# iamwangyabin/hardnetNas

Measured on AMD Instinct MI355X. Metric: Mpatches/s (32×32→128-D) at 1/2/4/8 MI355X; HPatches FPR95 parity, higher is better.
Workload: dtype bf16x3; 1 GPU; Stock HardNet forward, 262144 synthetic 32x32 patches per GPU; model=hardnet, global_batch=262144, per_gpu_batch=262144, parallelism=dp1

## Files before the change

### hardnetnas_amd/csrc/hn_api.hip

```cpp
#include "hardnet_mi355x.h"
#include "hn_internal.h"

#include <algorithm>
#include <cmath>
#include <cstdlib>
#include <cstring>
#include <map>
#include <mutex>
#include <string>
#include <utility>
#include <vector>

static thread_local std::string g_err;

static int env_int(const char* name, int dflt) {
  const char* e = std::getenv(name);
  return e ? std::atoi(e) : dflt;
}

void hn_read_knobs(HnKnobs* k) {
  *k = HnKnobs{};
  k->c12_cfg = env_int("HN_C12_CFG", 15);
  k->head = std::getenv("HN_HEAD_V1") ? 1 : env_int("HN_HEAD", 4);
  k->head_pf = env_int("HN_HEAD_PF", 1) != 0;
  k->fdl_valu = std::getenv("HN_FDL_VALU") != nullptr;
  k->naive_pw = std::getenv("HN_NAIVE_PW") != nullptr;
  k->naive_dw = std::getenv("HN_NAIVE_DW") != nullptr;
  k->no_skipfuse = std::getenv("HN_NO_SKIPFUSE") != nullptr;
  k->no_irfskip = std::getenv("HN_NO_IRFSKIP") != nullptr;
  k->pairdist_valu = std::getenv("HN_PAIRDIST_VALU") != nullptr;
  k->pairdist_reg = env_int("HN_PAIRDIST_REG", 0) != 0;
  k->pairdist_spread = env_int("HN_PAIRDIST_SPREAD", 1) != 0;
  k->front_fold = env_int("HN_FRONT_FOLD", 0) != 0;
  k->u8_apart = env_int("HN_U8_APART", 0) != 0;
  k->front_xch3 = env_int("HN_FRONT_XCH3", 0) != 0;
  k->no_mpfront = env_int("HN_NO_MPFRONT", 0) != 0;
  k->pipeline = env_int("HN_PIPELINE", 0) != 0;

  k->train_splitk = std::max(32, env_int("HN_TRAIN_SPLITK", 1024)) / 32 * 32;
  k->train_f32 = env_int("HN_TRAIN_F32", 17) & 255;
#ifdef HN_EXPERIMENTS
  k->c12_abl = env_int("HN_C12_ABL", 0) & 4095;
  k->c12w_pd = env_int("HN_C12W_PD", 11);
  k->dbg = env_int("HN_DEBUG", 0);
  k->head_abl = env_int("HN_HEAD_ABL", 0);
  k->w4_abl = env_int("HN_W4_ABL", 0);
  k->pairdist_abl = env_int("HN_PAIRDIST_ABL", 0);
  k->irf3 = env_int("HN_IRF3", 0) != 0;
#endif
}

static thread_local const HnKnobs* tl_knobs = nullptr;

const HnKnobs& hn_knobs() {
  if (tl_knobs) return *tl_knobs;
  static std::once_flag once;
  static HnKnobs process;
  std::call_once(once, [] { hn_read_knobs(&process); });
  return process;
}

namespace {
struct KnobScope {
  const HnKnobs* prev;
  explicit KnobScope(const HnKnobs* k) : prev(tl_knobs) { tl_knobs = k; }
  ~KnobScope() { tl_knobs = prev; }
};
}

hipError_t hn_resident_blocks(const void* fn, int nthreads, int lds, int* resident) {
  static std::mutex mu;
  static std::map<std::pair<const void*, int>, int> cache;
  int dev = 0;
  hipError_t e = hipGetDevice(&dev);
// ... 159 lines not shown
  bool c12 = true;
  int subchunk = 65536;
  int c12group = 65536;
  int c4sub = 0;
  uint16_t* front_spack = nullptr;
  int front = 0;
  bool no_front = false;
  bool no_irf = false;
  bool no_irf2 = false;
  const HnConvRow* conv[6] = {};
  size_t ws_floats_per_patch = 0;
  int n_bufs = 0;
  hipStream_t st2 = nullptr;
  hipEvent_t ev_fork = nullptr, ev_ready[2] = {nullptr, nullptr}, ev_free[2] = {nullptr, nullptr};
  std::mutex pipe_mu;

  template <class T>
  int upload(const std::vector<T>& v, T** out) {
    void* d = nullptr;
    if (hipMalloc(&d, v.size() * sizeof(T)) != hipSuccess)
      return fail(HN_ERR_NOMEM, "hipMalloc of parameters failed");
    allocs.push_back(d);
    HIPCHK(hipMemcpy(d, v.data(), v.size() * sizeof(T), hipMemcpyHostToDevice));
    *out = static_cast<T*>(d);
    return HN_OK;
  }
  ~hn_model() {
    for (void* p : allocs) (void)hipFree(p);
    for (hipEvent_t e : {ev_fork, ev_ready[0], ev_ready[1], ev_free[0], ev_free[1]})
      if (e) (void)hipEventDestroy(e);
    if (st2) (void)hipStreamDestroy(st2);
  }
};

static int check_desc(const hn_arch_desc* d) {
  if (!d) return fail(HN_ERR_ARG, "desc is NULL");
  if (d->kind == HN_KIND_HARDNET) return HN_OK;
  const bool fdl = d->kind == HN_KIND_FDL_NASNET || d->kind == HN_KIND_FDL_NASNET01;
  if (d->kind != HN_KIND_NAS && !fdl) return fail(HN_ERR_ARG, "unknown desc->kind");
  if (d->n_layers < 1 || d->n_layers > HN_MAX_LAYERS)
    return fail(HN_ERR_ARG, "n_layers out of range");
  int hw = fdl ? 8 : 32, c = fdl ? 64 : 32;
  for (int i = 0; i < d->n_layers; ++i) {
    if (d->op[i] < 0 || d->op[i] >= 17) return fail(HN_ERR_ARG, "op index out of range");
    if (d->c_in[i] != c) return fail(HN_ERR_ARG, "c_in does not chain");
    if (d->stride[i] != 1 && d->stride[i] != 2) return fail(HN_ERR_ARG, "stride must be 1/2");
    if (d->c_out[i] % 4 || d->c_in[i] % 4 || d->c_out[i] > 256)
      return fail(HN_ERR_ARG, "channel counts must be multiples of 4 and <= 256");
// ... 588 lines not shown
  (void)hipGetDevice(&m->device);
  Cursor cur{host_params, n_params};
  tl_f16_out_of_range = 0;
  rc = desc->kind == HN_KIND_HARDNET ? build_hardnet(m, cur)
       : desc->kind == HN_KIND_NAS    ? build_nas(m, cur)
                                      : build_fdl(m, cur);
  if (!rc && cur.i != n_params) rc = fail(HN_ERR_ARG, "host_params not fully consumed");
  if (!rc && tl_f16_out_of_range)
    rc = fail(HN_ERR_ARG, std::to_string(tl_f16_out_of_range) +
                              " BN-folded weights are outside the fp16 range of the fp16x3 kernels (|w| >= 65520 "
                              "or not finite)");
  if (rc) {
    delete m;
    return rc;
  }
  *out = m;
  return HN_OK;
}

static bool hardnet_subchunked(const hn_model* m) {
  return m->desc.kind == HN_KIND_HARDNET && m->c12 && !m->unfused_stem;
}
static int64_t hardnet_sub(const hn_model* m, int64_t p) { return std::max<int64_t>(1, std::min<int64_t>(p, m->subchunk)); }
static int64_t hardnet_group(const hn_model* m, int64_t p) {
  return std::max(hardnet_sub(m, p), std::min<int64_t>(p, m->c12group));
}
static size_t hardnet_a3_floats(const hn_model* m, int64_t p) {
  return std::max((size_t)16384 * hardnet_sub(m, p), (size_t)8192 * std::min<int64_t>(p, kHeadSplitMaxP));
}

// ... 262 lines not shown
extern "C" int hn_forward(hn_model* m, const float* d_in, int64_t batch, float* d_out,
                          void* d_workspace, size_t workspace_bytes, void* hip_stream) {
  if (!m) return fail(HN_ERR_ARG, "model is NULL");
  if (batch < 0) return fail(HN_ERR_ARG, "negative batch");
  if (batch == 0) return HN_OK;
  if (!d_in || !d_out || !d_workspace) return fail(HN_ERR_ARG, "NULL device pointer");
  if ((reinterpret_cast<uintptr_t>(d_in) | reinterpret_cast<uintptr_t>(d_out) |
       reinterpret_cast<uintptr_t>(d_workspace)) & 15)
    return fail(HN_ERR_ARG, "device pointers must be 16-byte aligned");
  size_t need = 0;
  hn_workspace_bytes(m, batch, &need);
  if (workspace_bytes < need)
    return fail(HN_ERR_WORKSPACE, "workspace too small: need " + std::to_string(need) + " bytes");
  hipStream_t st = static_cast<hipStream_t>(hip_stream);
  KnobScope knobs(&m->knobs);
  if (hardnet_pipelined(m, batch)) return forward_hardnet_pipe(m, d_in, batch, d_out, static_cast<float*>(d_workspace), st);
  for (int64_t off = 0; off < batch; off += m->chunk) {
    const int P = (int)std::min<int64_t>(m->chunk, batch - off);
    const float* in = d_in + off * 1024;
    float* out = d_out + off * 128;
    float* ws = static_cast<float*>(d_workspace);
    const int pmax = (int)std::min<int64_t>(m->chunk, batch);
    const int rc = m->desc.kind == HN_KIND_HARDNET ? forward_hardnet(m, in, P, pmax, out, ws, st)
                                                   : forward_nas(m, in, P, pmax, out, ws, st);
    if (rc) return rc;
  }
  return HN_OK;
}

static bool u8_fused(const hn_model* m, int resize) {
// ... 25 lines not shown
  if (in_hw != want)
    return fail(HN_ERR_ARG, "in_hw must be " + std::to_string(want) + " for this resize mode, got " +
                                std::to_string(in_hw));
  if (normalize && !(stdv != 0.0f)) return fail(HN_ERR_ARG, "std must be nonzero");
  if (batch == 0) return HN_OK;
  if (!d_in || !d_out || !d_workspace) return fail(HN_ERR_ARG, "NULL device pointer");
  if ((reinterpret_cast<uintptr_t>(d_in) | reinterpret_cast<uintptr_t>(d_out) |
       reinterpret_cast<uintptr_t>(d_workspace)) & 15)
    return fail(HN_ERR_ARG, "device pointers must be 16-byte aligned");
  size_t need = 0;
  hn_workspace_bytes_u8(m, batch, &need);
  if (workspace_bytes < need)
    return fail(HN_ERR_WORKSPACE, "workspace too small: need " + std::to_string(need) + " bytes");
  hipStream_t st = static_cast<hipStream_t>(hip_stream);
  KnobScope knobs(&m->knobs);
  const bool fused = u8_fused(m, resize);
  const size_t inb = (size_t)in_hw * in_hw;
  float* ws = static_cast<float*>(d_workspace);
  size_t base = 0;
  hn_workspace_bytes(m, batch, &base);
  float* pre = reinterpret_cast<float*>(static_cast<char*>(d_workspace) + base);
  const int pmax = (int)std::min<int64_t>(m->chunk, batch);
  for (int64_t off = 0; off < batch; off += m->chunk) {
    const int P = (int)std::min<int64_t>(m->chunk, batch - off);
    const uint8_t* in = d_in + off * inb;
    float* out = d_out + off * 128;
    int rc;
    if (fused) {
      const HnU8In u8{in, resize, normalize, mean, stdv};
      rc = m->desc.kind == HN_KIND_HARDNET ? forward_hardnet(m, nullptr, P, pmax, out, ws, st, &u8)
// ... 41 lines not shown
                             const int64_t* d_kpts, const float* d_scale, const float* d_ori, const float* d_ratio,
                             int64_t n, float* d_out, void* d_workspace, size_t workspace_bytes, void* hip_stream) {
  if (const char* e = clip_arg_error(n_images, height, width, n)) return fail(HN_ERR_ARG, e);
  if (!m) return fail(HN_ERR_ARG, "model is NULL");
  if (n == 0) return HN_OK;
  if (!d_images || !d_kpts || !d_scale || !d_ratio || !d_out || !d_workspace)
    return fail(HN_ERR_ARG, "NULL device pointer (only d_ori may be NULL)");
  if ((reinterpret_cast<uintptr_t>(d_out) | reinterpret_cast<uintptr_t>(d_workspace)) & 15)
    return fail(HN_ERR_ARG, "d_out / d_workspace must be 16-byte aligned");
  size_t need = 0, base = 0;
  hn_workspace_bytes_kp(m, n, &need);
  if (workspace_bytes < need)
    return fail(HN_ERR_WORKSPACE, "workspace too small: need " + std::to_string(need) + " bytes");
  hipStream_t st = static_cast<hipStream_t>(hip_stream);
  KnobScope knobs(&m->knobs);
  float* ws = static_cast<float*>(d_workspace);
  hn_workspace_bytes(m, n, &base);
  float* patches = reinterpret_cast<float*>(static_cast<char*>(d_workspace) + base);
  const int pmax = (int)std::min<int64_t>(m->chunk, n);
  for (int64_t off = 0; off < n; off += m->chunk) {
    const int P = (int)std::min<int64_t>(m->chunk, n - off);
    STAGE("clip", hn_launch_clip(d_images, n_images, height, width, d_kpts + off * 4, d_scale + off,
                                 d_ori ? d_ori + off * 2 : nullptr, d_ratio, P, patches, st));
    const int rc = m->desc.kind == HN_KIND_HARDNET ? forward_hardnet(m, patches, P, pmax, d_out + off * 128, ws, st)
                                                   : forward_nas(m, patches, P, pmax, d_out + off * 128, ws, st);
    if (rc) return rc;
  }
  return HN_OK;
}

// ... 594 lines not shown
```

### hardnetnas_amd/csrc/hn_hardnet.hip

```cpp
#include "hn_common.h"
#include "hn_internal.h"

#include <algorithm>
#include <cstdlib>

template <bool NORM>
__global__ __launch_bounds__(256) void k_stem(const float* __restrict__ in, float* __restrict__ out,
                                              const float* __restrict__ w,
                                              const float* __restrict__ b,
                                              float eps) {
  __shared__ float tile[34 * 34];
  __shared__ float red[8];
  const int t = threadIdx.x;
  const size_t p = blockIdx.x;
  const float4 v = reinterpret_cast<const float4*>(in + p * 1024)[t];
  for (int i = t; i < 34 * 34; i += 256) tile[i] = 0.f;
  float mean = 0.f, sd = 1.f;
  if (NORM) {
    float s = wave_sum(v.x + v.y + v.z + v.w);
    if ((t & 63) == 0) red[t >> 6] = s;
    __syncthreads();
    mean = (red[0] + red[1] + red[2] + red[3]) * (1.f / 1024.f);
    const float d0 = v.x - mean, d1 = v.y - mean, d2 = v.z - mean, d3 = v.w - mean;
    float q = wave_sum(d0 * d0 + d1 * d1 + d2 * d2 + d3 * d3);
// ... 653 lines not shown
  using C = WsCfg<CIN, COUT, HIN, S, NP, TR, WM, WN, STEM, PX, CST, PST>;
  static_assert(PX == 80 || !STEM, "the stem producer writes the 80-byte layout");
  extern __shared__ __attribute__((aligned(16))) char smem[];
  const int tid = threadIdx.x, lane = tid & 63;
  const int wave = __builtin_amdgcn_readfirstlane(tid >> 6);
  const bool producer = wave >= C::NWC;
  const int r = lane & 31, h = lane >> 5;
  const int nwg = gridDim.x, rb = xcd_remap(blockIdx.x, nwg);
  const int ntiles = (P + NP - 1) / NP * C::RT;
  const int per = (ntiles + nwg - 1) / nwg;
  const int t_begin = STEM ? rb * per : rb;
  const int my_tiles = STEM ? max(0, min(per, ntiles - t_begin))
                            : (rb < ntiles ? (ntiles - 1 - rb) / nwg + 1 : 0);
  const int NS = my_tiles * C::NCC;
  if (NS == 0) return;
  char* const buf0 = smem;
  char* const buf1 = smem + C::BUF;
  auto stage_at = [&](const char* b, int m) -> char* {
    return m < C::MB ? const_cast<char*>(b) + m * C::OSTR : smem + C::BIAS_OFF + COUT * 4 + (m - C::MB) * C::OSTR;
  };

  auto tile_of = [&](int s, int& p0, int& y0) {
    const int t = STEM ? t_begin + s / C::NCC : rb + (s / C::NCC) * nwg;
    p0 = (t / C::RT) * NP;
    y0 = (t % C::RT) * TR;
  };
  const int ptid = tid - C::NWC * 64;
  float4 pf[C::UPT][2], pf2[C::UPT][2];
  auto produce_loads = [&](int s, float4 (&pf)[C::UPT][2]) {
    int p0, y0;
// ... 355 lines not shown
#pragma unroll
            for (int k = 0; k < 4; ++k) {
              const int pl = 8 * k + (lane >> 3), c4 = lane & 7;
              *reinterpret_cast<float4*>(ob + (size_t)pl * COUT + 4 * c4) =
                  *reinterpret_cast<const float4*>(scr + pl * C::SROW + 4 * c4);
            }
            __builtin_amdgcn_wave_barrier();
            asm volatile("" ::: "memory");
          }
        }
      }
      if constexpr (!(ABL & 32)) __syncthreads();
    }
  }
  if constexpr (PST) __builtin_amdgcn_s_barrier();
}

template <int K>
__global__ __launch_bounds__(256) void k_head(const float* __restrict__ a, float* __restrict__ out,
                                              const uint4* __restrict__ wp,
                                              const float* __restrict__ bias, int P, float l2eps) {
  __shared__ float ssq[2][64];
  const int tid = threadIdx.x, lane = tid & 63, wave = tid >> 6;
  const int wm = wave >> 1, wn = wave & 1;
  const int r = lane & 31, h = lane >> 5;
  const int pbase = blockIdx.x * 64 + wm * 32;
  const int pa = min(pbase + r, P - 1);
  const float* arow = a + (size_t)pa * K + h * 8;
  f32x16 acc[2] = {f32x16{}, f32x16{}};
#pragma unroll 4
// ... 617 lines not shown
    {3, 7, row<3, Ws<64, 64, 16, 1, 1, 16, 4, 1, false, 0, 80, false, false>>},
    {4, 7, row<4, Ws<64, 128, 16, 2, 1, 8, 2, 2, false, 0, 80, false, false>>},
    {5, 7, row<5, Ws<128, 128, 8, 1, 2, 8, 2, 2, false, 0, 80, false, false>>},
    {4, 13, row<4, Ws<64, 128, 16, 2, 2, 8, 1, 4, false, 0, 64, false, false>>},
    {4, 14, row<4, Ws<64, 128, 16, 2, 1, 8, 1, 4, false, 0, 64, false, false>>},
    {3, 18, row<3, Ws<64, 64, 16, 1, 1, 16, 2, 2, false, 0, 80, false, true>>},
    {3, 8, row<3, Ws<64, 64, 16, 1, 1, 16, 2, 2, false, 45, 80, false, false>>},
    {4, 8, row<4, Ws<64, 128, 16, 2, 1, 8, 1, 4, false, 45, 80, false, false>>},
    {5, 8, row<5, Ws<128, 128, 8, 1, 2, 8, 1, 4, false, 45, 80, false, false>>},
    {3, 9, row<3, Ws<64, 64, 16, 1, 1, 16, 2, 2, false, 8, 80, false, false>>},
    {4, 9, row<4, Ws<64, 128, 16, 2, 1, 8, 1, 4, false, 8, 80, false, false>>},
    {5, 9, row<5, Ws<128, 128, 8, 1, 2, 8, 1, 4, false, 8, 80, false, false>>},
    {3, 4, row<3, Ws<64, 64, 16, 1, 1, 16, 2, 2, false, 40, 80, false, false>>},
    {4, 4, row<4, Ws<64, 128, 16, 2, 1, 8, 1, 4, false, 40, 80, false, false>>},
    {5, 4, row<5, Ws<128, 128, 8, 1, 2, 8, 1, 4, false, 40, 80, false, false>>},
#endif
};
static_assert(hn_rows_unique(kConvRows), "one build per (layer, HN_VARIANT digit)");

}

hipError_t hn_launch_stem(const float* in, float* out, const float* w, const float* b, int P,
                          bool norm, float eps, hipStream_t st) {
  if (norm)
    hipLaunchKernelGGL(k_stem<true>, dim3(P), dim3(256), 0, st, in, out, w, b, eps);
  else
    hipLaunchKernelGGL(k_stem<false>, dim3(P), dim3(256), 0, st, in, out, w, b, eps);
  return hipGetLastError();
}

// ... 101 lines not shown
```

### hardnetnas_amd/csrc/hn_internal.h

```cpp
#pragma once
#include <hip/hip_runtime.h>

#include <algorithm>
#include <type_traits>

#include "hardnet_mi355x.h"

struct HnKnobs {
  int c12_cfg = 15;
  int head = 4;
  bool head_pf = true;
  bool fdl_valu = false;
  bool naive_pw = false;
  bool naive_dw = false;
  bool no_skipfuse = false;
  bool no_irfskip = false;
  bool pairdist_valu = false;
  bool pairdist_reg = false;
  bool pairdist_spread = true;
  bool front_fold = false;
  bool u8_apart = false;
  bool front_xch3 = false;
  bool no_mpfront = false;
  bool pipeline = false;
  bool irf3 = false;
  int train_splitk = 1024;
  int train_f32 = 17;
  int c12w_pd = 11;
  int c12_abl = 0;
  int head_abl = 0;
  int w4_abl = 0;
  int pairdist_abl = 0;
  int dbg = 0;
};
void hn_read_knobs(HnKnobs* k);
const HnKnobs& hn_knobs();

hipError_t hn_resident_blocks(const void* fn, int nthreads, int lds, int* resident);

struct HardnetDev {
  float* stem_w = nullptr;
  float* stem_b = nullptr;
  void* wpack[7] = {};
  float* bias[7] = {};
  void* c12_w1 = nullptr;
  void* c12_w2 = nullptr;
  void* c12_w1w = nullptr;
  void* wino[7] = {};
  void* wino1[7] = {};
  void* wino4[7] = {};
};
// ... 269 lines not shown
```

### hardnetnas_amd/csrc/hn_wino1.hip

```cpp
#include "hn_common.h"
#include "hn_internal.h"

namespace {

template <int CIN, int COUT, int H, int NP, int WM, int WN, bool CST>
struct W1Cfg {
  static constexpr int TR = H;
  static constexpr int NTX = H / 2;
  static constexpr int BM = NP * TR * NTX;
  static constexpr int MT = BM / WM / 32, NT = COUT / WN / 32;
  static constexpr int NTOT = COUT / 32, NCC = CIN / 32;
  static constexpr int XROW = NTX * 64;
  static constexpr int RS = 4 * XROW;
  static constexpr int PS = TR * RS;
  static constexpr int ZROW = NP * PS;
  static constexpr int PLANE = ZROW + RS;
  static constexpr int BUF = 2 * PLANE;
  static constexpr int NWC = WM * WN, NWP = 4, NTHR = (NWC + NWP) * 64, PTHR = NWP * 64;
  static constexpr int UNITS = NP * TR * NTX * 4;
  static_assert(64 % (4 * NTX) == 0 && PTHR % (4 * NTX) == 0, "a row's units share one wave");
  static constexpr int UPT = (UNITS + PTHR - 1) / PTHR;
  static constexpr bool DEEP = UPT <= 2;
  static constexpr int SROW = 36;
  static constexpr int SCR_OFF = 2 * BUF;
  static constexpr int SCR = CST ? 32 * SROW * 4 : 0;
  static constexpr int BIAS_OFF = SCR_OFF + NWC * SCR;
  static constexpr int SMEM = BIAS_OFF + COUT * 4;
  static constexpr int NKS = 24;
  static constexpr unsigned CHUNK_BYTES = NKS * NTOT * 2 * 64 * 16;
  static_assert(SMEM <= 160 * 1024, "LDS");
  static_assert(MT >= 1 && NT >= 1 && MT * WM * 32 == BM && NT * WN * 32 == COUT, "tiling");
  static_assert((TR * NTX) % 32 == 0 && 32 % NTX == 0, "an M tile = 32 / NTX whole rows of one patch");
  static_assert(RS % 256 == 0, "image rows on 256-byte boundaries (the bank-conflict argument)");
};

template <int... I, class F>
HN_DEV void static_for_seq(std::integer_sequence<int, I...>, F&& f) {
  (f(std::integral_constant<int, I>{}), ...);
}
template <int N, class F>
HN_DEV void static_for(F&& f) {
  static_for_seq(std::make_integer_sequence<int, N>{}, f);
}

constexpr int w1_lo3(int g) { return g == 0 ? 0 : g == 1 ? 6 : g == 2 ? 11 : 16; }
constexpr int w1_fold_valu(bool first, int kx, int g) {
  if (kx == 11 && g >= 3) return 2 * (w1_lo3(g - 2) - w1_lo3(g - 3));
  if (kx == 12 && g < 3) return 2 * (w1_lo3(g + 1) - w1_lo3(g));
  if (kx == 18 || kx == 19 || (kx == 0 && !first)) return g < 5 ? 3 : 1;
  if (kx == 23 && g >= 3) return w1_lo3(g - 2) - w1_lo3(g - 3);
  return 0;
}

template <int CIN, int COUT, int H, int NP, int WM, int WN, bool CST, int WD = 3, int ABL = 0>
__global__ __launch_bounds__((WM * WN + 4) * 64) void k_conv_w1(const float* __restrict__ in, float* __restrict__ out,
                                                                const uint4* __restrict__ wp,
                                                                const float* __restrict__ bias, int P) {
  using C = W1Cfg<CIN, COUT, H, NP, WM, WN, CST>;
  constexpr int TR = C::TR;
  extern __shared__ __attribute__((aligned(16))) char smem[];
  const int tid = threadIdx.x, lane = tid & 63;
  const int wave = __builtin_amdgcn_readfirstlane(tid >> 6);
  const bool producer = wave >= C::NWC;
  const int r = lane & 31, h = lane >> 5;
  const int nwg = gridDim.x, rb = xcd_remap(blockIdx.x, nwg);
  const int ntiles = (P + NP - 1) / NP;
  const int my_tiles = rb < ntiles ? (ntiles - 1 - rb) / nwg + 1 : 0;
  const int NS = my_tiles * C::NCC;
  if (NS == 0) return;
  char* const buf0 = smem;
  char* const buf1 = smem + C::BUF;
  auto tile_of = [&](int s) { return (rb + (s / C::NCC) * nwg) * NP; };

  const int ptid = tid - C::NWC * 64;
  float4 pf[C::UPT][6], pf2[C::UPT][6];
  constexpr unsigned PATCH_BYTES = (unsigned)H * H * CIN * 4, OOB = 0x80000000u;
  auto produce_loads = [&](int s, float4 (&d)[C::UPT][6]) {
    const bool live = s < NS;
    const int p0 = live ? tile_of(s) : 0;
    const int cc = s % C::NCC;
    const int nval = !live ? 0 : P - p0 < NP ? P - p0 : NP;
    const __amdgpu_buffer_rsrc_t rs = make_rsrc(in + (size_t)p0 * H * H * CIN, (unsigned)nval * PATCH_BYTES);
#pragma unroll
    for (int k = 0; k < C::UPT; ++k) {
      const int u = ptid + k * C::PTHR;
      const int g = u & 3, t = (u >> 2) % C::NTX, rest = (u >> 2) / C::NTX;
      const int y = rest % TR, np = rest / TR;
      const bool rowok = C::UNITS % C::PTHR == 0 || u < C::UNITS;
#pragma unroll
      for (int j = 0; j < 3; ++j) {
        const int x = 2 * t - 1 + j;
        const bool ok = rowok && (j < 2 || t == C::NTX - 1) && (unsigned)x < (unsigned)H;
        const unsigned vo = ok ? (unsigned)(((np * H + y) * H + x) * CIN + cc * 32 + g * 8) * 4u : OOB;
        d[k][2 * j] = __builtin_bit_cast(float4, buf_load16(rs, vo, 0));
        d[k][2 * j + 1] = __builtin_bit_cast(float4, buf_load16(rs, vo, 16));
// ... 30 lines not shown
          for (int i = 0; i < 2; ++i) {
            const float4 d0 = dd[0][i], d1 = dd[1][i], d2 = dd[2][i], d3 = dd[3][i];
            if (xi == 0) v[i] = make_float4(d0.x - d2.x, d0.y - d2.y, d0.z - d2.z, d0.w - d2.w);
            if (xi == 1) v[i] = make_float4(d1.x + d2.x, d1.y + d2.y, d1.z + d2.z, d1.w + d2.w);
            if (xi == 2) v[i] = make_float4(d2.x - d1.x, d2.y - d1.y, d2.z - d1.z, d2.w - d1.w);
            if (xi == 3) v[i] = make_float4(d1.x - d3.x, d1.y - d3.y, d1.z - d3.z, d1.w - d3.w);
          }
          uint4 hi, lo;
          split8(v[0], v[1], hi, lo);
          *reinterpret_cast<uint4*>(dst + off + xi * C::XROW) = hi;
          *reinterpret_cast<uint4*>(dst + C::PLANE + off + xi * C::XROW) = lo;
        }
      }
    }
  };

  for (int i = tid; i < 4 * C::RS / 16; i += C::NTHR) {
    const int q = i / (C::RS / 16), o = (i % (C::RS / 16)) * 16;
    *reinterpret_cast<uint4*>(smem + (q >> 1) * C::BUF + (q & 1) * C::PLANE + C::ZROW + o) = make_uint4(0, 0, 0, 0);
  }
  if constexpr ((ABL & 64) != 0) {
    if (!producer) __builtin_amdgcn_s_setprio(1);
  }
  if constexpr ((ABL & 128) != 0) {
    if (producer) __builtin_amdgcn_s_setprio(1);
  }
  if (producer) {
    if constexpr ((ABL & 1) != 0) {
#pragma unroll 1
      for (int s = 0; s <= NS; ++s) __syncthreads();
      return;
    }
    produce_loads(0, pf);
    produce_write(buf0, pf);
    produce_loads(1, pf);
    __syncthreads();
    if constexpr (!C::DEEP) {
#pragma unroll 1
      for (int s = 0; s < NS; ++s) {
        produce_write((s & 1) ? buf0 : buf1, pf);
        produce_loads(s + 2, pf);
        __syncthreads();
      }
    } else {
#pragma unroll 1
// ... 126 lines not shown
            fold(first_, kx_, g_);
            __builtin_amdgcn_sched_group_barrier(0x008, 1, 0);
            __builtin_amdgcn_sched_group_barrier(0x002, nv, 0);
          } else if constexpr (w1_fold_valu(FIRST, kx, 0) + w1_fold_valu(FIRST, kx, 5) > 0) {
            __builtin_amdgcn_sched_group_barrier(0x008, 1, 0);
          }
        }
      });
      __builtin_amdgcn_sched_barrier(0);
    });
  };
  auto fold_last = [&] {
#pragma unroll
    for (int i = 0; i < 16; ++i) y1a[1][i] = ssub(y1a[1][i], ma[1][i]);
  };
#pragma unroll 1
  for (int t = 0; t < my_tiles; ++t) {
    const int s0 = t * C::NCC, s = s0 + C::NCC - 1;
    stage(std::true_type{}, s0, 0, C::NCC > 1 ? 1 : 0);
#pragma unroll 1
    for (int cc = 1; cc < C::NCC; ++cc) {
      __syncthreads();
      stage(std::false_type{}, s0 + cc, cc, (cc + 1) % C::NCC);
    }
    if constexpr ((ABL & 2) == 0) fold_last();
    {
      const int p0 = tile_of(s);
      int le = lane;
      asm volatile("" : "+v"(le));
      const int r = le & 31, h = le >> 5;
#pragma unroll
      for (int nt = 0; nt < C::NT; ++nt) {
        float4 bv[4];
#pragma unroll
        for (int q = 0; q < 4; ++q)
          bv[q] = *reinterpret_cast<const float4*>(sbias + (wn * C::NT + nt) * 32 + 8 * q + 4 * h);
#pragma unroll
        for (int mt = 0; mt < C::MT; ++mt) {
          const int m0 = (wm * C::MT + mt) * 32;
          const int np = m0 / (TR * C::NTX), yb = (m0 % (TR * C::NTX)) / C::NTX;
          if ((NP == 1 || p0 + np < P) && ((ABL & 8) == 0 || y0a[mt * C::NT + nt][0] == 1234.5f)) {
            float* const ob = out + (((size_t)p0 + np) * H + yb) * H * COUT + (wn * C::NT + nt) * 32;
// ... 20 lines not shown
                }
                __builtin_amdgcn_wave_barrier();
                asm volatile("" ::: "memory");
              } else {
                const int px = (r / C::NTX) * H + 2 * (r % C::NTX) + par;
#pragma unroll
                for (int q = 0; q < 4; ++q)
                  *reinterpret_cast<float4*>(ob + (size_t)px * COUT + 8 * q + 4 * h) = v[q];
              }
            }
          }
        }
      }
    }
    __syncthreads();
  }
}

template <int L, int CIN, int COUT, int H, int NP, int WM, int WN, bool CST, int WD, int ABL>
hipError_t launch_w1(const HardnetDev& d, const float* in, float* out, int P, float, hipStream_t st) {
  using C = W1Cfg<CIN, COUT, H, NP, WM, WN, CST>;
  if (!d.wino1[L]) return hipErrorInvalidValue;
  return hn_launch_persistent<&k_conv_w1<CIN, COUT, H, NP, WM, WN, CST, WD, ABL>, C::NTHR, C::SMEM>(
      (P + NP - 1) / NP, st, in, out, static_cast<const uint4*>(d.wino1[L]), d.bias[L], P);
}

#ifdef HN_EXPERIMENTS
template <int CIN, int COUT, int H, int NP, int WN>
struct W4Cfg {
  static constexpr int NTX = H / 4;
  static constexpr int POS = NP * H * NTX;
  static constexpr int MT = POS / 16;
  static constexpr int NCC = CIN / 32;
  static constexpr int NT = COUT / 16 / WN;
  static constexpr int RB = NTX * 64;
  static constexpr int HR = H + 2;
  static constexpr int XB = HR * RB;
  static constexpr int PLANE = NP * 6 * XB;
  static constexpr int BUF = 2 * PLANE;
// ... 333 lines not shown
    {5, 23, w1c5<8, 2>},
    {3, 24, w1c3<8, 4>},
    {5, 24, w1c5<8, 4>},
    {3, 25, w1c3<8, 8>},
    {5, 25, w1c5<8, 8>},
    {3, 29, w1c3<8, 16>},
    {5, 29, w1c5<8, 16>},
    {3, 30, w1c3<8, 32>},
    {5, 30, w1c5<8, 32>},
    {3, 31, w1c3<8, 34>},
    {5, 31, w1c5<8, 34>},
    {3, 34, w1c3<8, 64>},
    {5, 34, w1c5<8, 64>},
    {3, 35, w1c3<8, 128>},
    {5, 35, w1c5<8, 128>},
    {3, 32, launch_w4c3<6>},
    {3, 33, launch_w4c3<9>},
#endif
};
static_assert(hn_rows_unique(kWino1Rows), "one build per (layer, HN_VARIANT digit)");

}

const HnConvRow* hn_wino1_conv_row(int layer, int variant) { return hn_find_row(kWino1Rows, layer, variant); }


int hn_wino1_lds_bytes(int layer) {
  switch (layer) {
    case 3: return W1Conv3::SMEM;
    case 5: return W1Conv5::SMEM;
// ... 4 lines not shown
```

### include/hardnet_mi355x.h

```cpp
#ifndef HARDNET_MI355X_H
#define HARDNET_MI355X_H

#include <stddef.h>
#include <stdint.h>

#ifdef __cplusplus
extern "C" {
#endif

#define HN_ABI_VERSION 2

enum hn_status {
  HN_OK = 0,
  HN_ERR_ARG = 1,
  HN_ERR_HIP = 2,
  HN_ERR_NOMEM = 3,
  HN_ERR_WORKSPACE = 4
};

enum hn_kind {
  HN_KIND_HARDNET = 0,
  HN_KIND_NAS = 1,
  HN_KIND_FDL_NASNET = 2,
  HN_KIND_FDL_NASNET01 = 3,
// ... 9 lines not shown
  int32_t c_in[HN_MAX_LAYERS];
  int32_t c_out[HN_MAX_LAYERS];
  int32_t stride[HN_MAX_LAYERS];
  float input_norm_eps;
  float l2_eps;
  float bn_eps;
} hn_arch_desc;

typedef struct hn_model hn_model;

int hn_param_count(const hn_arch_desc* desc, size_t* n_out);

int hn_create(const hn_arch_desc* desc, const float* host_params, size_t n_params,
              hn_model** out);

int hn_workspace_bytes(const hn_model* m, int64_t batch, size_t* bytes_out);

int hn_forward(hn_model* m, const float* d_in, int64_t batch, float* d_out,
               void* d_workspace, size_t workspace_bytes, void* hip_stream);

int hn_pairdist_workspace_bytes(int64_t batch, size_t* bytes_out);
int hn_pairdist_hardneg(const float* d_anchor, const float* d_positive, int64_t batch, int32_t dim,
                        int32_t anchor_swap, float* d_pos, float* d_min_neg,
                        void* d_workspace, size_t workspace_bytes, void* hip_stream);

int hn_pairdist_rows_workspace_bytes(int64_t n_rows, int64_t batch, size_t* bytes_out);
int hn_pairdist_rows(const float* d_anchor_rows, int64_t n_rows, int64_t row0, const float* d_positive,
                     int64_t batch, int32_t dim, float* d_pos, float* d_row_min, float* d_col_min,
                     void* d_workspace, size_t workspace_bytes, void* hip_stream);

// ... 104 lines not shown
```

Baseline: 5.788 Mpatches/s.

## Add dynamic tile claiming via atomic counters to persistent Winograd conv kernels

Persistent Winograd conv3/conv5 kernels can now claim tiles dynamically through a global atomic counter instead of using a fixed round-robin assignment. The producer warps keep a small LDS ring of upcoming tile indices and reset the counter when the last workgroup finishes. Per-forward counter blocks come from a ring of device allocations, with separate slots for graph capture. The aim is to reduce tail imbalance across workgroups, at the cost of atomics, extra LDS, and more complex synchronisation. The change also adds timestamp probes and a host-side invariant checker.

```diff
diff --git a/hardnetnas_amd/csrc/hn_api.hip b/hardnetnas_amd/csrc/hn_api.hip
--- a/hardnetnas_amd/csrc/hn_api.hip
+++ b/hardnetnas_amd/csrc/hn_api.hip
@@ -2,6 +2,7 @@
 #include "hn_internal.h"
 
 #include <algorithm>
+#include <atomic>
 #include <cmath>
 #include <cstdlib>
 #include <cstring>
@@ -36,6 +37,7 @@
   k->front_xch3 = env_int("HN_FRONT_XCH3", 0) != 0;
   k->no_mpfront = env_int("HN_NO_MPFRONT", 0) != 0;
   k->pipeline = env_int("HN_PIPELINE", 0) != 0;
+  k->dyn_tiles = env_int("HN_STATIC_TILES", 0) != 0 ? 0 : env_int("HN_DYN_TILES", 3) & (kTilesConv3 | kTilesConv5);
 
   k->train_splitk = std::max(32, env_int("HN_TRAIN_SPLITK", 1024)) / 32 * 32;
   k->train_f32 = env_int("HN_TRAIN_F32", 17) & 255;
@@ -58,6 +60,14 @@
   static HnKnobs process;
   std::call_once(once, [] { hn_read_knobs(&process); });
   return process;
+}
+
+static thread_local unsigned* tl_tile_block = nullptr;
+static thread_local unsigned tl_tile_launch = 0;
+
+unsigned* hn_tile_counters(int kernel) {
+  if (!tl_tile_block || !(hn_knobs().dyn_tiles & kernel)) return nullptr;
+  return tl_tile_block + 2 * (tl_tile_launch++ % kTileLaunches);
 }
 
 namespace {
@@ -247,6 +257,8 @@
   hipStream_t st2 = nullptr;
   hipEvent_t ev_fork = nullptr, ev_ready[2] = {nullptr, nullptr}, ev_free[2] = {nullptr, nullptr};
   std::mutex pipe_mu;
+  unsigned* tile_ctrs = nullptr;
+  std::atomic<unsigned> tile_next{0}, tile_captures{0};
 
   template <class T>
   int upload(const std::vector<T>& v, T** out) {
@@ -265,6 +277,37 @@
     if (st2) (void)hipStreamDestroy(st2);
   }
 };
+
+namespace {
+struct TileScope {
+  unsigned* prev_block;
+  unsigned prev_launch;
+  TileScope(hn_model* m, hipStream_t st) : prev_block(tl_tile_block), prev_launch(tl_tile_launch) {
+    tl_tile_block = nullptr;
+    tl_tile_launch = 0;
+    if (!m->tile_ctrs || !m->knobs.dyn_tiles) return;
+    hipStreamCaptureStatus cs = hipStreamCaptureStatusNone;
+    if (hipStreamIsCapturing(st, &cs) != hipSuccess) {
+      (void)hipGetLastError();
+      cs = hipStreamCaptureStatusNone;
+    }
+    unsigned b;
+    if (cs != hipStreamCaptureStatusNone) {
+      if (m->tile_captures.load() >= HN_TILE_CAPTURES) return;
+      b = m->tile_captures.fetch_add(1);
+      if (b >= HN_TILE_CAPTURES) return;
+      b += HN_TILE_RING;
+    } else {
+      b = m->tile_next.fetch_add(1) % HN_TILE_RING;
+    }
+    tl_tile_block = m->tile_ctrs + (size_t)b * 2 * kTileLaunches;
+  }
+  ~TileScope() {
+    tl_tile_block = prev_block;
+    tl_tile_launch = prev_launch;
+  }
+};
+}
 
 static int check_desc(const hn_arch_desc* d) {
   if (!d) return fail(HN_ERR_ARG, "desc is NULL");
@@ -883,6 +926,19 @@
     delete m;
     return rc;
   }
+  if (desc->kind == HN_KIND_HARDNET && m->knobs.dyn_tiles) {
+    const size_t bytes = (size_t)(HN_TILE_RING + HN_TILE_CAPTURES) * kTileLaunches * 2 * sizeof(unsigned);
+    void* p = nullptr;
+    if (hipMalloc(&p, bytes) == hipSuccess) {
+      if (hipMemset(p, 0, bytes) == hipSuccess && hipDeviceSynchronize() == hipSuccess) {
+        m->allocs.push_back(p);
+        m->tile_ctrs = static_cast<unsigned*>(p);
+      } else {
+        (void)hipFree(p);
+      }
+    }
+    if (!m->tile_ctrs) (void)hipGetLastError();
+  }
   *out = m;
   return HN_OK;
 }
@@ -1175,6 +1231,7 @@
     return fail(HN_ERR_WORKSPACE, "workspace too small: need " + std::to_string(need) + " bytes");
   hipStream_t st = static_cast<hipStream_t>(hip_stream);
   KnobScope knobs(&m->knobs);
+  TileScope tiles(m, st);
   if (hardnet_pipelined(m, batch)) return forward_hardnet_pipe(m, d_in, batch, d_out, static_cast<float*>(d_workspace), st);
   for (int64_t off = 0; off < batch; off += m->chunk) {
     const int P = (int)std::min<int64_t>(m->chunk, batch - off);
@@ -1230,6 +1287,7 @@
     return fail(HN_ERR_WORKSPACE, "workspace too small: need " + std::to_string(need) + " bytes");
   hipStream_t st = static_cast<hipStream_t>(hip_stream);
   KnobScope knobs(&m->knobs);
+  TileScope tiles(m, st);
   const bool fused = u8_fused(m, resize);
   const size_t inb = (size_t)in_hw * in_hw;
   float* ws = static_cast<float*>(d_workspace);
@@ -1301,6 +1359,7 @@
     return fail(HN_ERR_WORKSPACE, "workspace too small: need " + std::to_string(need) + " bytes");
   hipStream_t st = static_cast<hipStream_t>(hip_stream);
   KnobScope knobs(&m->knobs);
+  TileScope tiles(m, st);
   float* ws = static_cast<float*>(d_workspace);
   hn_workspace_bytes(m, n, &base);
   float* patches = reinterpret_cast<float*>(static_cast<char*>(d_workspace) + base);
diff --git a/hardnetnas_amd/csrc/hn_hardnet.hip b/hardnetnas_amd/csrc/hn_hardnet.hip
--- a/hardnetnas_amd/csrc/hn_hardnet.hip
+++ b/hardnetnas_amd/csrc/hn_hardnet.hip
@@ -691,6 +691,11 @@
                             : (rb < ntiles ? (ntiles - 1 - rb) / nwg + 1 : 0);
   const int NS = my_tiles * C::NCC;
   if (NS == 0) return;
+  long long* const stamps = reinterpret_cast<long long*>(const_cast<float*>(in) + (size_t)P * 40960 + (2 << 20) / 4) +
+                            1024 + 2 * blockIdx.x;
+  if constexpr ((ABL & 64) != 0) {
+    if (tid == 0) stamps[0] = (long long)__builtin_amdgcn_s_memrealtime();
+  }
   char* const buf0 = smem;
   char* const buf1 = smem + C::BUF;
   auto stage_at = [&](const char* b, int m) -> char* {
@@ -1076,6 +1081,9 @@
     }
   }
   if constexpr (PST) __builtin_amdgcn_s_barrier();
+  if constexpr ((ABL & 64) != 0) {
+    if (tid == 0) stamps[1] = (long long)__builtin_amdgcn_s_memrealtime();
+  }
 }
 
 template <int K>
@@ -1723,6 +1731,7 @@
     {3, 4, row<3, Ws<64, 64, 16, 1, 1, 16, 2, 2, false, 40, 80, false, false>>},
     {4, 4, row<4, Ws<64, 128, 16, 2, 1, 8, 1, 4, false, 40, 80, false, false>>},
     {5, 4, row<5, Ws<128, 128, 8, 1, 2, 8, 1, 4, false, 40, 80, false, false>>},
+    {4, 27, row<4, Ws<64, 128, 16, 2, 2, 8, 2, 2, false, 64, 64, false, true>>},
 #endif
 };
 static_assert(hn_rows_unique(kConvRows), "one build per (layer, HN_VARIANT digit)");
diff --git a/hardnetnas_amd/csrc/hn_internal.h b/hardnetnas_amd/csrc/hn_internal.h
--- a/hardnetnas_amd/csrc/hn_internal.h
+++ b/hardnetnas_amd/csrc/hn_internal.h
@@ -24,6 +24,7 @@
   bool no_mpfront = false;
   bool pipeline = false;
   bool irf3 = false;
+  int dyn_tiles = 3;
   int train_splitk = 1024;
   int train_f32 = 17;
   int c12w_pd = 11;
@@ -35,6 +36,10 @@
 };
 void hn_read_knobs(HnKnobs* k);
 const HnKnobs& hn_knobs();
+
+constexpr int kTilesConv3 = 1, kTilesConv5 = 2;
+constexpr int kTileLaunches = 32;
+unsigned* hn_tile_counters(int kernel);
 
 hipError_t hn_resident_blocks(const void* fn, int nthreads, int lds, int* resident);
 
diff --git a/hardnetnas_amd/csrc/hn_tiles.h b/hardnetnas_amd/csrc/hn_tiles.h
--- /dev/null
+++ b/hardnetnas_amd/csrc/hn_tiles.h
@@ -0,0 +1,87 @@
+#pragma once
+
+#if defined(__HIPCC__)
+#define HN_TILES_FN __host__ __device__ inline
+#else
+#define HN_TILES_FN inline
+#endif
+
+namespace hn_tiles {
+
+constexpr int kEnd = -1;
+constexpr int kAhead = 2;
+constexpr int kSlots = 4;
+
+HN_TILES_FN int slot(int k) { return k & (kSlots - 1); }
+
+HN_TILES_FN int fixed_tile(int k, int rb, int nwg, int ntiles) {
+  const long long t = (long long)rb + (long long)k * nwg;
+  return t < ntiles ? (int)t : kEnd;
+}
+HN_TILES_FN int claimed_tile(unsigned v, int nwg, int ntiles) {
+  const long long t = (long long)kAhead * nwg + v;
+  return t < ntiles ? (int)t : kEnd;
+}
+
+struct Claimer {
+  bool live;
+  unsigned ticket;
+  bool left;
+  unsigned before;
+};
+HN_TILES_FN Claimer claimer(bool claiming_lane) { return Claimer{claiming_lane, 0u, false, 0u}; }
+template <class Ctr>
+HN_TILES_FN void claim_issue(Claimer& c, Ctr& ctr) {
+  if (c.live) c.ticket = ctr.take();
+}
+template <class Ctr>
+HN_TILES_FN int claim_settle(Claimer& c, Ctr& ctr, int nwg, int ntiles) {
+  if (!c.live) return kEnd;
+  const int t = claimed_tile(c.ticket, nwg, ntiles);
+  if (t == kEnd) {
+    c.live = false;
+    c.left = true;
+    c.before = ctr.leave();
+  }
+  return t;
+}
+template <class Ctr>
+HN_TILES_FN void claim_finish(Claimer& c, Ctr& ctr, int nwg) {
+  if (c.left && c.before == (unsigned)nwg - 1u) ctr.reset();
+}
+HN_TILES_FN void ring_init(int* ring, int rb, int nwg, int ntiles) {
+  for (int k = 0; k < kAhead; ++k) ring[slot(k)] = fixed_tile(k, rb, nwg, ntiles);
+}
+
+struct Cursor {
+  int k;
+  int cur;
+  int nxt;
+};
+HN_TILES_FN void cursor_start(Cursor& c, const int* ring) {
+  c.k = 0;
+  c.cur = ring[slot(0)];
+  c.nxt = ring[slot(1)];
+}
+HN_TILES_FN bool cursor_done(const Cursor& c) { return c.cur == kEnd; }
+HN_TILES_FN void cursor_advance(Cursor& c, const int* ring) {
+  ++c.k;
+  c.cur = c.nxt;
+  c.nxt = ring[slot(c.k + 1)];
+}
+HN_TILES_FN int stage_tile(const Cursor& c, int j, int ncc) { return j < ncc ? c.cur : c.nxt; }
+HN_TILES_FN int stage_chunk(int j, int ncc) { return j < ncc ? j : j - ncc; }
+
+#if defined(__HIPCC__)
+struct DeviceCounter {
+  unsigned* p;
+  __device__ unsigned take() { return atomicAdd(p, 1u); }
+  __device__ unsigned leave() { return atomicAdd(p + 1, 1u); }
+  __device__ void reset() {
+    atomicExch(p, 0u);
+    atomicExch(p + 1, 0u);
+  }
+};
+#endif
+
+}
diff --git a/hardnetnas_amd/csrc/hn_tiles_host_check.cpp b/hardnetnas_amd/csrc/hn_tiles_host_check.cpp
--- /dev/null
+++ b/hardnetnas_amd/csrc/hn_tiles_host_check.cpp
@@ -0,0 +1,229 @@
+#include <algorithm>
+#include <cstdio>
+#include <cstdlib>
+#include <random>
+#include <utility>
+#include <vector>
+
+#include "hn_tiles.h"
+
+namespace {
+
+using namespace hn_tiles;
+
+#define CHECK(cond, ...)                       \
+  do {                                         \
+    if (!(cond)) {                             \
+      std::fprintf(stderr, "FAILED %s: ", #cond); \
+      std::fprintf(stderr, __VA_ARGS__);       \
+      std::fprintf(stderr, "\n");              \
+      std::exit(1);                            \
+    }                                          \
+  } while (0)
+
+struct MockCounter {
+  unsigned next = 0, left = 0;
+  long takes = 0;
+  unsigned take() {
+    ++takes;
+    return next++;
+  }
+  unsigned leave() { return left++; }
+  void reset() { next = left = 0; }
+};
+
+struct Ring {
+  int word[kSlots];
+  int tag[kSlots];
+  Ring() {
+    for (int i = 0; i < kSlots; ++i) word[i] = 12345, tag[i] = -1000;
+  }
+};
+
+using Stage = std::pair<int, int>;
+
+struct Role {
+  bool producer = false;
+  int rb = 0, nwg = 0, ntiles = 0, ncc = 0;
+  Ring* ring = nullptr;
+  MockCounter* ctr = nullptr;
+  Claimer cl = claimer(false);
+  Cursor c{0, 0, 0};
+  int arrived = 0;
+  bool finished = false;
+  int pc = 0, j = 0;
+  std::vector<int> tiles;
+  std::vector<Stage> stages;
+
+  void check_tags(int k) {
+    CHECK(ring->tag[slot(k)] == k, "rb %d %s: T_%d read, slot holds T_%d", rb, producer ? "producer" : "mfma", k,
+          ring->tag[slot(k)]);
+    CHECK(ring->tag[slot(k + 1)] == k + 1, "rb %d %s: T_%d read, slot holds T_%d", rb, producer ? "producer" : "mfma",
+          k + 1, ring->tag[slot(k + 1)]);
+  }
+  void stage_for(int s_local) {
+    const int t = stage_tile(c, s_local, ncc), cc = stage_chunk(s_local, ncc);
+    const size_t s = (size_t)c.k * ncc + s_local;
+    if (stages.size() <= s) stages.resize(s + 1, Stage(-7, -7));
+    stages[s] = Stage(t, cc);
+  }
+  bool step() {
+    if (producer) {
+      switch (pc) {
+        case 0:
+          ring_init(ring->word, rb, nwg, ntiles);
+          for (int k = 0; k < kAhead; ++k) ring->tag[slot(k)] = k;
+          stages.push_back(Stage(rb, 0));
+          pc = 1;
+          return true;
+        case 1:
+          check_tags(0);
+          cursor_start(c, ring->word);
+          pc = 2;
+          [[fallthrough]];
+        case 2:
+          if (cursor_done(c)) {
+            claim_finish(cl, *ctr, nwg);
+            return false;
+          }
+          tiles.push_back(c.cur);
+          if (c.k == 0) stage_for(1);
+          claim_issue(cl, *ctr);
+          j = 0;
+          [[fallthrough]];
+        case 3:
+          stage_for(j + 2);
+          pc = 4;
+          return true;
+        case 4: {
+          if (j + 3 < 2 * ncc) stage_for(j + 3);
+          const bool last = j + 2 == ncc;
+          if (last) {
+            const int t = claim_settle(cl, *ctr, nwg, ntiles);
+            CHECK(ring->tag[slot(c.k + 2)] == c.k + 2 - kSlots || ring->tag[slot(c.k + 2)] == -1000,
+                  "rb %d: publishing T_%d over T_%d", rb, c.k + 2, ring->tag[slot(c.k + 2)]);
+            ring->word[slot(c.k + 2)] = t;
+            ring->tag[slot(c.k + 2)] = c.k + 2;
+          }
+          j += 2;
+          pc = last ? 5 : 3;
+          return true;
+        }
+        case 5:
+          check_tags(c.k + 1);
+          cursor_advance(c, ring->word);
+          pc = 2;
+          return step();
+      }
+    } else {
+      switch (pc) {
+        case 0:
+          pc = 1;
+          return true;
+        case 1:
+          check_tags(0);
+          cursor_start(c, ring->word);
+          pc = 2;
+          [[fallthrough]];
+        case 2:
+          if (cursor_done(c)) return false;
+          tiles.push_back(c.cur);
+          j = 0;
+          [[fallthrough]];
+        case 3:
+          stages.push_back(Stage(c.cur, j));
+          ++j;
+          pc = j == ncc ? 5 : 3;
+          return true;
+        case 5:
+          check_tags(c.k + 1);
+          cursor_advance(c, ring->word);
+          pc = 2;
+          return step();
+      }
+    }
+    CHECK(false, "bad pc %d", pc);
+    return false;
+  }
+};
+
+long run_launch(int W, int ntiles, int ncc, MockCounter& ctr, std::mt19937& rng) {
+  const int nwg = std::min(W, ntiles);
+  if (nwg == 0) return 0;
+  const long takes0 = ctr.takes;
+  std::vector<int> perm(nwg);
+  for (int i = 0; i < nwg; ++i) perm[i] = i;
+  std::shuffle(perm.begin(), perm.end(), rng);
+  std::vector<Ring> rings(nwg);
+  std::vector<Role> roles(2 * nwg);
+  for (int w = 0; w < nwg; ++w)
+    for (int r = 0; r < 2; ++r) {
+      Role& x = roles[2 * w + r];
+      x.producer = r == 0;
+      x.rb = perm[w];
+      x.nwg = nwg;
+      x.ntiles = ntiles;
+      x.ncc = ncc;
+      x.ring = &rings[w];
+      x.ctr = &ctr;
+      x.cl = claimer(x.producer);
+    }
+  std::vector<int> runnable;
+  for (;;) {
+    runnable.clear();
+    bool all_done = true;
+    for (int i = 0; i < 2 * nwg; ++i) {
+      const Role &x = roles[i], &o = roles[i ^ 1];
+      if (x.finished) continue;
+      all_done = false;
+      if (x.arrived <= o.arrived) runnable.push_back(i);
+      else CHECK(!o.finished, "rb %d: a role waits at barrier %d, its partner ended after %d", x.rb, x.arrived, o.arrived);
+    }
+    if (all_done) break;
+    CHECK(!runnable.empty(), "deadlock");
+    const int i = runnable[rng() % runnable.size()];
+    Role& x = roles[i];
+    if (x.step()) ++x.arrived;
+    else x.finished = true;
+  }
+  std::vector<int> seen(ntiles, 0);
+  for (int w = 0; w < nwg; ++w) {
+    const Role &p = roles[2 * w], &m = roles[2 * w + 1];
+    CHECK(p.arrived == m.arrived, "rb %d: %d producer barriers, %d MFMA barriers", p.rb, p.arrived, m.arrived);
+    CHECK(p.tiles == m.tiles, "rb %d: the roles' tile sequences differ", p.rb);
+    CHECK(p.arrived == 1 + ncc * (int)m.tiles.size(), "rb %d: barrier count", p.rb);
+    CHECK(p.stages.size() >= m.stages.size(), "rb %d: stages staged", p.rb);
+    for (size_t s = 0; s < m.stages.size(); ++s)
+      CHECK(p.stages[s] == m.stages[s], "rb %d stage %zu: staged (%d, %d), computed (%d, %d)", p.rb, s, p.stages[s].first,
+            p.stages[s].second, m.stages[s].first, m.stages[s].second);
+    for (size_t s = m.stages.size(); s < p.stages.size(); ++s)
+      CHECK(p.stages[s].first == kEnd, "rb %d: stage %zu staged for tile %d and never computed", p.rb, s, p.stages[s].first);
+    CHECK(!p.cl.live && p.cl.left, "rb %d: the claimer never checked out", p.rb);
+    for (int t : m.tiles) {
+      CHECK(t >= 0 && t < ntiles, "rb %d: tile %d of %d", p.rb, t, ntiles);
+      ++seen[t];
+    }
+  }
+  for (int t = 0; t < ntiles; ++t) CHECK(seen[t] == 1, "tile %d of %d run %d times (W %d)", t, ntiles, seen[t], W);
+  CHECK(ctr.next == 0 && ctr.left == 0, "counters end at %u / %u (W %d, ntiles %d)", ctr.next, ctr.left, W, ntiles);
+  return ctr.takes - takes0;
+}
+
+}
+
+int main() {
+  std::mt19937 rng(20240611u);
+  long launches = 0, takes = 0;
+  for (int W : {1, 2, 3, 5, 8, 13})
+    for (int ncc : {2, 4})
+      for (int ntiles = 0; ntiles <= 5 * W + 3; ++ntiles)
+        for (int rep = 0; rep < 24; ++rep) {
+          MockCounter ctr;
+          for (int launch = 0; launch < 2; ++launch) {
+            takes += run_launch(W, ntiles, ncc, ctr, rng);
+            ++launches;
+          }
+        }
+  std::printf("hn_tiles host check: %ld launches, %ld claims, all invariants held\n", launches, takes);
+  return 0;
+}
diff --git a/hardnetnas_amd/csrc/hn_wino1.hip b/hardnetnas_amd/csrc/hn_wino1.hip
--- a/hardnetnas_amd/csrc/hn_wino1.hip
+++ b/hardnetnas_amd/csrc/hn_wino1.hip
@@ -1,5 +1,6 @@
 #include "hn_common.h"
 #include "hn_internal.h"
+#include "hn_tiles.h"
 
 namespace {
 
@@ -25,7 +26,8 @@
   static constexpr int SCR_OFF = 2 * BUF;
   static constexpr int SCR = CST ? 32 * SROW * 4 : 0;
   static constexpr int BIAS_OFF = SCR_OFF + NWC * SCR;
-  static constexpr int SMEM = BIAS_OFF + COUT * 4;
+  static constexpr int TQ_OFF = BIAS_OFF + COUT * 4;
+  static constexpr int SMEM = TQ_OFF + hn_tiles::kSlots * 4;
   static constexpr int NKS = 24;
   static constexpr unsigned CHUNK_BYTES = NKS * NTOT * 2 * 64 * 16;
   static_assert(SMEM <= 160 * 1024, "LDS");
@@ -52,11 +54,15 @@
   return 0;
 }
 
-template <int CIN, int COUT, int H, int NP, int WM, int WN, bool CST, int WD = 3, int ABL = 0>
+template <int CIN, int COUT, int H, int NP, int WM, int WN, bool CST, int WD = 3, int ABL = 0, bool DYN = false>
 __global__ __launch_bounds__((WM * WN + 4) * 64) void k_conv_w1(const float* __restrict__ in, float* __restrict__ out,
                                                                 const uint4* __restrict__ wp,
-                                                                const float* __restrict__ bias, int P) {
+                                                                const float* __restrict__ bias, int P,
+                                                                unsigned* __restrict__ tile_ctr,
+                                                                long long* __restrict__ stamps) {
   using C = W1Cfg<CIN, COUT, H, NP, WM, WN, CST>;
+  static_assert(!DYN || ((ABL & ~256) == 0 && C::DEEP && C::NCC % 2 == 0),
+                "claimed tiles: the two-stage producer body, whole bodies per tile, no ablation");
   constexpr int TR = C::TR;
   extern __shared__ __attribute__((aligned(16))) char smem[];
   const int tid = threadIdx.x, lane = tid & 63;
@@ -68,17 +74,21 @@
   const int my_tiles = rb < ntiles ? (ntiles - 1 - rb) / nwg + 1 : 0;
   const int NS = my_tiles * C::NCC;
   if (NS == 0) return;
+  if constexpr ((ABL & 256) != 0) {
+    if (tid == 0) stamps[2 * blockIdx.x] = (long long)__builtin_amdgcn_s_memrealtime();
+  }
   char* const buf0 = smem;
   char* const buf1 = smem + C::BUF;
+  int* const tq = reinterpret_cast<int*>(smem + C::TQ_OFF);
   auto tile_of = [&](int s) { return (rb + (s / C::NCC) * nwg) * NP; };
 
   const int ptid = tid - C::NWC * 64;
   float4 pf[C::UPT][6], pf2[C::UPT][6];
   constexpr unsigned PATCH_BYTES = (unsigned)H * H * CIN * 4, OOB = 0x80000000u;
-  auto produce_loads = [&](int s, float4 (&d)[C::UPT][6]) {
-    const bool live = s < NS;
-    const int p0 = live ? tile_of(s) : 0;
-    const int cc = s % C::NCC;
+  auto produce_loads_at = [&](int tile, int cc, float4 (&d)[C::UPT][6]) {
+    if constexpr (DYN) tile = __builtin_amdgcn_readfirstlane(tile);
+    const bool live = tile != hn_tiles::kEnd;
+    const int p0 = live ? tile * NP : 0;
     const int nval = !live ? 0 : P - p0 < NP ? P - p0 : NP;
     const __amdgpu_buffer_rsrc_t rs = make_rsrc(in + (size_t)p0 * H * H * CIN, (unsigned)nval * PATCH_BYTES);
 #pragma unroll
@@ -139,6 +149,9 @@
       }
     }
   };
+  auto produce_loads = [&](int s, float4 (&d)[C::UPT][6]) {
+    produce_loads_at(s < NS ? rb + (s / C::NCC) * nwg : hn_tiles::kEnd, s % C::NCC, d);
+  };
 
   for (int i = tid; i < 4 * C::RS / 16; i += C::NTHR) {
     const int q = i / (C::RS / 16), o = (i % (C::RS / 16)) * 16;
@@ -154,6 +167,40 @@
     if constexpr ((ABL & 1) != 0) {
 #pragma unroll 1
       for (int s = 0; s <= NS; ++s) __syncthreads();
+      return;
+    }
+    if constexpr (DYN) {
+      hn_tiles::DeviceCounter ctr{tile_ctr};
+      hn_tiles::Claimer cl = hn_tiles::claimer(ptid == 0);
+      if (ptid == 0) hn_tiles::ring_init(tq, rb, nwg, ntiles);
+      produce_loads_at(rb, 0, pf);
+      produce_write(buf0, pf);
+      produce_loads_at(rb, 1, pf);
+      __syncthreads();
+      hn_tiles::Cursor c;
+      hn_tiles::cursor_start(c, tq);
+      c.cur = __builtin_amdgcn_readfirstlane(c.cur);
+      c.nxt = __builtin_amdgcn_readfirstlane(c.nxt);
+#pragma unroll 1
+      while (!hn_tiles::cursor_done(c)) {
+        hn_tiles::claim_issue(cl, ctr);
+#pragma unroll 1
+        for (int j = 0; j < C::NCC; j += 2) {
+          produce_loads_at(hn_tiles::stage_tile(c, j + 2, C::NCC), hn_tiles::stage_chunk(j + 2, C::NCC), pf2);
+          produce_write(buf1, pf);
+          __syncthreads();
+          produce_loads_at(hn_tiles::stage_tile(c, j + 3, C::NCC), hn_tiles::stage_chunk(j + 3, C::NCC), pf);
+          produce_write(buf0, pf2);
+          if (j + 2 == C::NCC) {
+            const int t = hn_tiles::claim_settle(cl, ctr, nwg, ntiles);
+            if (ptid == 0) tq[hn_tiles::slot(c.k + 2)] = t;
+          }
+          __syncthreads();
+        }
+        hn_tiles::cursor_advance(c, tq);
+        c.nxt = __builtin_amdgcn_readfirstlane(c.nxt);
+      }
+      hn_tiles::claim_finish(cl, ctr, nwg);
       return;
     }
     produce_loads(0, pf);
@@ -310,9 +357,14 @@
 #pragma unroll
     for (int i = 0; i < 16; ++i) y1a[1][i] = ssub(y1a[1][i], ma[1][i]);
   };
-#pragma unroll 1
-  for (int t = 0; t < my_tiles; ++t) {
-    const int s0 = t * C::NCC, s = s0 + C::NCC - 1;
+  hn_tiles::Cursor c{0, 0, 0};
+  if constexpr (DYN) {
+    hn_tiles::cursor_start(c, tq);
+    c.cur = __builtin_amdgcn_readfirstlane(c.cur);
+  }
+#pragma unroll 1
+  for (int t = 0; DYN ? !hn_tiles::cursor_done(c) : t < my_tiles; ++t) {
+    const int s0 = DYN ? 0 : t * C::NCC, s = s0 + C::NCC - 1;
     stage(std::true_type{}, s0, 0, C::NCC > 1 ? 1 : 0);
 #pragma unroll 1
     for (int cc = 1; cc < C::NCC; ++cc) {
@@ -321,7 +373,7 @@
     }
     if constexpr ((ABL & 2) == 0) fold_last();
     {
-      const int p0 = tile_of(s);
+      const int p0 = DYN ? c.cur * NP : tile_of(s);
       int le = lane;
       asm volatile("" : "+v"(le));
       const int r = le & 31, h = le >> 5;
@@ -372,6 +424,13 @@
       }
     }
     __syncthreads();
+    if constexpr (DYN) {
+      hn_tiles::cursor_advance(c, tq);
+      c.cur = __builtin_amdgcn_readfirstlane(c.cur);
+    }
+  }
+  if constexpr ((ABL & 256) != 0) {
+    if (tid == 0) stamps[2 * blockIdx.x + 1] = (long long)__builtin_amdgcn_s_memrealtime();
   }
 }
 
@@ -379,8 +438,18 @@
 hipError_t launch_w1(const HardnetDev& d, const float* in, float* out, int P, float, hipStream_t st) {
   using C = W1Cfg<CIN, COUT, H, NP, WM, WN, CST>;
   if (!d.wino1[L]) return hipErrorInvalidValue;
+  const uint4* w = static_cast<const uint4*>(d.wino1[L]);
+  long long* stamps = nullptr;
+  if constexpr ((ABL & 256) != 0)
+    stamps = reinterpret_cast<long long*>((L == 3 ? out + (size_t)P * 40960 : const_cast<float*>(in) + (size_t)P * 24576) +
+                                          (2 << 20) / 4) + (L == 3 ? 0 : 2048);
+  if constexpr ((ABL & ~256) == 0) {
+    if (unsigned* ctr = hn_tile_counters(L == 3 ? kTilesConv3 : kTilesConv5))
+      return hn_launch_persistent<&k_conv_w1<CIN, COUT, H, NP, WM, WN, CST, WD, ABL, true>, C::NTHR, C::SMEM>(
+          (P + NP - 1) / NP, st, in, out, w, d.bias[L], P, ctr, stamps);
+  }
   return hn_launch_persistent<&k_conv_w1<CIN, COUT, H, NP, WM, WN, CST, WD, ABL>, C::NTHR, C::SMEM>(
-      (P + NP - 1) / NP, st, in, out, static_cast<const uint4*>(d.wino1[L]), d.bias[L], P);
+      (P + NP - 1) / NP, st, in, out, w, d.bias[L], P, (unsigned*)nullptr, stamps);
 }
 
 #ifdef HN_EXPERIMENTS
@@ -744,6 +813,8 @@
     {5, 34, w1c5<8, 64>},
     {3, 35, w1c3<8, 128>},
     {5, 35, w1c5<8, 128>},
+    {3, 27, w1c3<8, 256>},
+    {5, 27, w1c5<6, 256>},
     {3, 32, launch_w4c3<6>},
     {3, 33, launch_w4c3<9>},
 #endif
diff --git a/include/hardnet_mi355x.h b/include/hardnet_mi355x.h
--- a/include/hardnet_mi355x.h
+++ b/include/hardnet_mi355x.h
@@ -47,6 +47,8 @@
 int hn_create(const hn_arch_desc* desc, const float* host_params, size_t n_params,
               hn_model** out);
 
+#define HN_TILE_RING 64
+#define HN_TILE_CAPTURES 64
 int hn_workspace_bytes(const hn_model* m, int64_t batch, size_t* bytes_out);
 
 int hn_forward(hn_model* m, const float* d_in, int64_t batch, float* d_out,
```

New measurement: 5.876 Mpatches/s (median of 6 runs). +1.5%, better.
